# rueberger/MJHMC

Hardware: AMD Instinct MI355X
Metric: particle-steps/sec (ndims x nparticles x L) (higher is better)
Workload: dtype f64 state (ProductOfT: around the f32 matrix-core force)

## Files before the change

### mjhmc_amd/csrc/api.hip

```cpp
#include <hip/hip_runtime.h>

#include <cmath>
#include <cstdio>
#include <functional>
#include <vector>

#include "autocor.hpp"
#include "lagcov.hpp"
#include "sampler_internal.hpp"

static thread_local std::string g_err;

int mjhmc_fail(int code, const std::string& msg) {
  g_err = msg;
  return code;
}
const std::string& last_error_text() { return g_err; }


int pick_shape(int D, int dtype, Shape* out) {
  const int esize = dtype == MJHMC_F64 ? 8 : 4;
  const int VEC = 16 / esize;
  Shape s;
  s.esize = esize;
// ... 467 lines not shown
    if (q) (void)hipFree(q);
  for (void* q : e->sic)
    if (q) (void)hipFree(q);
  delete e;
  return 0;
}

int mjhmc_sampler_destroy(mjhmc_sampler* s) {
  if (!s) return 0;
  (void)hipSetDevice(s->ctx->device);
  if (s->stream) (void)hipStreamSynchronize(s->stream);
  functionals_free_all(s);
  accumulators_free_all(s);
  timegrid_free_all(s);
  stein_free_all(s);
  void* ptrs[] = {s->flf_list, s->call_block, s->Hpre, s->Hwork, s->cold_list, s->pot64_scratch, s->Hspec[0], s->Hspec[1], s->Hspec_dump, s->Gbuf[0], s->Gbuf[1], s->Xbuf[0], s->Xbuf[1], s->Vbuf[0],  s->Vbuf[1], s->EX[0],     s->EX[1],  s->EV[0],
                  s->EV[1],   s->Hflf[0], s->Hflf[1],  s->dwell,  s->dwell_scratch,  s->trans,
                  s->ring,     s->dwell_ring, s->stage,  s->noise,  s->rexp,
                  s->runif,   s->scratch,  s->ck[0],    s->ck[1],    s->ck[2],   s->ck[3],  s->ck[4],
                  s->ck[5],   s->ck[6]};
  for (void* p : ptrs)
    if (p) (void)hipFree(p);
  for (auto& e : s->ev_total)
    if (e) (void)hipEventDestroy(e);
  for (auto& e : s->ev_k) (void)hipEventDestroy(e);
  for (auto& e : s->part_events) (void)hipEventDestroy(e);
  for (auto& q : s->part_streams) (void)hipStreamDestroy(q);
  if (s->ev_join) (void)hipEventDestroy(s->ev_join);
  if (s->ev_fork) (void)hipEventDestroy(s->ev_fork);
  for (void* q : s->ick)
    if (q) (void)hipFree(q);
// ... 44 lines not shown
    const size_t mb = mat_bytes(s);
    for (int i = 0; i < 2; ++i) {
      HIPCHK(hipMalloc(&s->Xbuf[i], mb));
      HIPCHK(hipMalloc(&s->Vbuf[i], mb));
      HIPCHK(hipMemsetAsync(s->Xbuf[i], 0, mb, s->stream));
      HIPCHK(hipMemsetAsync(s->Vbuf[i], 0, mb, s->stream));
      if (e->is_pot() || ((e->is_host() || s->sh.wide) && i == 0)) {
        HIPCHK(hipMalloc(&s->Gbuf[i], mb));
        HIPCHK(hipMemsetAsync(s->Gbuf[i], 0, mb, s->stream));
      }
      if (e->is_dense()) {
        if (!s->Hwork) {
          HIPCHK(hipMalloc((void**)&s->Hwork, s->Npad * ssize(s)));
          HIPCHK(hipMemsetAsync(s->Hwork, 0, s->Npad * ssize(s), s->stream));
          HIPCHK(hipMalloc((void**)&s->cold_list, (2 * s->Npad + 3 * kMaxDenseParts) * sizeof(int)));
          if (e->is_pot() && dtype == MJHMC_F64 && !e->pot_big() && !e->lin_tall())
            HIPCHK(hipMalloc((void**)&s->pot64_scratch, (size_t)kMaxDenseParts * pot64_scratch_workgroups() * 2 * 32 * row_bytes(s)));
        }
        HIPCHK(hipMalloc(&s->Hspec[i], s->Npad * ssize(s)));
        HIPCHK(hipMemsetAsync(s->Hspec[i], 0xFF, s->Npad * ssize(s), s->stream));
      }
      HIPCHK(hipMalloc(&s->EX[i], s->Npad * ssize(s)));
      HIPCHK(hipMalloc(&s->EV[i], s->Npad * ssize(s)));
      HIPCHK(hipMalloc(&s->Hflf[i], s->Npad * ssize(s)));
      HIPCHK(hipMemsetAsync(s->EX[i], 0, s->Npad * ssize(s), s->stream));
      HIPCHK(hipMemsetAsync(s->EV[i], 0, s->Npad * ssize(s), s->stream));
      HIPCHK(hipMemsetAsync(s->Hflf[i], 0xFF, s->Npad * ssize(s), s->stream));
    }
    HIPCHK(hipMalloc((void**)&s->dwell, s->Npad * sizeof(double)));
    HIPCHK(hipMemsetAsync(s->dwell, 0, s->Npad * sizeof(double), s->stream));
    HIPCHK(hipMalloc((void**)&s->dwell_scratch, s->Npad * sizeof(double)));
    HIPCHK(hipMalloc((void**)&s->trans, s->Npad));
// ... 232 lines not shown
```

### mjhmc_amd/csrc/dense_pot.hpp

```cpp
#pragma once
#ifndef __HIPCC_RTC__
#include <hip/hip_runtime.h>
#endif
#include <stdint.h>

#include "jump_math.hpp"
#include "jump_process.hpp"
#include "lane_group.hpp"
#include "philox.hpp"
#include "sampler_args.hpp"

namespace mjhmc {

constexpr int kPotDim = 512;

struct PotModel {
  const float* W1;
  const float* W2T;
  const float* cb;
  const float* alpha;
  int dim;
  int ndims;
};

// ... 142 lines not shown
  hipFunction_t jump32[3][2] = {};
  hipFunction_t jump64[3][2] = {};
  hipFunction_t eval = nullptr, leap = nullptr;
  PotLinear lin{};
};

void pot_launch_jump(const PotJumpArgs& a, const PotModel& mdl, hipStream_t st, const PotGenerated* gen = nullptr);
void pot_launch_eval(const PotEvalArgs& a, const PotModel& mdl, hipStream_t st, const PotGenerated* gen = nullptr);
void pot_launch_leap(const PotLeapArgs& a, const PotModel& mdl, hipStream_t st, const PotGenerated* gen = nullptr);
void pot64_launch_jump(const Pot64JumpArgs& a, const PotModel& mdl, hipStream_t st, const PotGenerated* gen = nullptr);
template <class A>
inline void pot_launch_generated(hipFunction_t f, unsigned grid, hipStream_t st, const A& a, const PotModel& mdl, const PotLinear& lin) {
  void* params[] = {(void*)&a, (void*)&mdl, (void*)&lin};
  (void)hipModuleLaunchKernel(f, grid, 1, 1, 256, 1, 1, 0, st, params, nullptr);
}
int pot64_scratch_workgroups();
#endif

}
```

### mjhmc_amd/csrc/dense_pot64.hip

```cpp
#include <hip/hip_runtime.h>
#include <stdint.h>

#include <algorithm>

#include "dense_pot.hpp"
#include "dense_pot64_kernels.hpp"
#include "dense_pot_tile.hpp"

namespace mjhmc {

__global__ void pot64_cold_list_kernel(const double* __restrict__ Hflf_in, const double* __restrict__ Hspec_in, int64_t N,
                                       int* __restrict__ list, int* __restrict__ count, const Control* ctl) {
  if (ctl->failed) return;
  const int64_t p = (int64_t)blockIdx.x * blockDim.x + threadIdx.x;
  const double hc = p < N ? Hflf_in[p] : 0.0, hs = p < N ? Hspec_in[p] : 0.0;
  append_cold(list, count, (p < N) && !(hc == hc) && !(hs == hs), p);
}

template <int NB, bool REPLAY, int MODE>
__global__ __launch_bounds__(256, 1) void pot64_jump_kernel(const Pot64JumpArgs a, const PotModel mdl) {
  const PotExperts xp;
#include "dense_pot64_jump.inc"
}

// ... 60 lines not shown
  if (n0) atomicAdd(&tally[0], n0);
  if (n1) atomicAdd(&tally[1], n1);
  if (n2) atomicAdd(&tally[2], n2);
  if (n3) atomicAdd(&tally[3], n3);
  __syncthreads();
  if (threadIdx.x < 4 && tally[threadIdx.x]) atomicAdd(&a.stats[threadIdx.x], (unsigned long long)tally[threadIdx.x]);
}

static int resident_cus64() {
  int dev = 0, cus = 0;
  (void)hipGetDevice(&dev);
  (void)hipDeviceGetAttribute(&cus, hipDeviceAttributeMultiprocessorCount, dev);
  return std::max(1, cus);
}

int pot64_scratch_workgroups() { return resident_cus64(); }

template <int NB, int MODE>
static void launch64_mode(const Pot64JumpArgs& a, const PotModel& mdl, unsigned grid, hipStream_t st, const PotGenerated* gen) {
  const bool replay = MODE == kModeControl ? (a.runif && a.noise) : (a.rexp && a.noise);
  if (gen) pot_launch_generated(gen->jump64[MODE][replay ? 1 : 0], grid, st, a, mdl, gen->lin);
  else if (replay) hipLaunchKernelGGL((pot64_jump_kernel<NB, true, MODE>), dim3(grid), dim3(256), 0, st, a, mdl);
  else hipLaunchKernelGGL((pot64_jump_kernel<NB, false, MODE>), dim3(grid), dim3(256), 0, st, a, mdl);
}

template <int NB>
static void launch64_nb(const Pot64JumpArgs& a, const PotModel& mdl, hipStream_t st, const PotGenerated* gen) {
  const int cus = resident_cus64();
  if (a.mode == kModeMJHMC) {
    if (a.iter == 0 || a.rescan) {
      (void)hipMemsetAsync(std::min(a.cold_count, std::min(a.next_count, a.zero_count)), 0, 3 * sizeof(int), st);
      hipLaunchKernelGGL(pot64_cold_list_kernel, dim3((unsigned)((a.N + 255) / 256)), dim3(256), 0, st, a.Hflf_in, a.Hspec_in,
// ... 33 lines not shown
```

### mjhmc_amd/csrc/dense_pot64_jump.inc

```
  __shared__ Shared64<NB> sh;
  if (a.ctl->failed) return;
  const int lane = threadIdx.x & 63, w = threadIdx.x >> 6, c = lane & 31, h = lane >> 5;
  const int ncold = MODE == kModeMJHMC ? *a.cold_count : 0;
  const int64_t nft = (ncold + kP - 1) / kP;
  if ((int64_t)blockIdx.x >= nft + a.ntiles) return;
  if (MODE == kModeMJHMC && blockIdx.x == 0 && threadIdx.x == 0) {
    *a.zero_count = 0;
    if (ncold) atomicAdd(&a.stats[3], (unsigned long long)ncold << 32);
  }
  __shared__ unsigned tally[5];
  if (threadIdx.x < 5) tally[threadIdx.x] = 0;
  AReg<NB> ar;
  areg_load<NB>(mdl, w, c, h, ar);
  stage_bias<NB>(mdl, sh.s);
  const Work<NB> wk = work_of<NB>(a.scratch, blockIdx.x, w, lane);
  for (int64_t item = blockIdx.x; item < nft + a.ntiles; item += gridDim.x) {
    const bool inverse = item < nft;
    [[maybe_unused]] const int istamp_item = (int)(item / gridDim.x) & 15;
    auto column_of = [&](int64_t it) -> int64_t {
      if (it < nft) {
        const int64_t slot = it * kP + c;
        return a.cold_list[slot < ncold ? slot : ncold - 1];
      }
      return (it - nft) * kP + c;
    };
    Tile<NB> g;
    VTile<NB> v;
    float exl = 0.f;
    double EVL;
    {
      const int64_t p = column_of(item);
      POT_ISTAMP(0);
      staged_start<NB>(sh.s, wk, a.X_in, a.V_in, a.G_in, p, w, c, h, g, v, inverse);
      POT_ISTAMP(1);
      EVL = pot64_trajectory<NB>(mdl, xp, ar, sh, w, c, h, lane, wk, g, v, a.L, a.eps, a.chalf, &exl);
      POT_ISTAMP(2);
    }
    int64_t item_again = item;
    asm volatile("" : "+s"(item_again));
    const int64_t p = column_of(item_again);
    const bool alive = p < a.N;
    const size_t roff = (size_t)p * (128 * NB) + 32 * NB * w + 4 * NB * h;
    if (!inverse) staged_end_x<NB>(sh.s, wk, a.X_out, p, w, c, h);
    POT_ISTAMP(3);
    const double EXL = (double)exl;
    const double HL = EXL + EVL;
    if (inverse) {
      if (w == 0 && h == 0) a.Hwork[p] = HL;
      __syncthreads();
      POT_ISTAMP(4);
      continue;
    }

    if constexpr (MODE == kModeMJHMC) {
      if (w == 0 && h == 0) {
        a.EX_out[p] = EXL;
        a.EV_out[p] = EVL;
      }
// ... 54 lines not shown
```

### mjhmc_amd/csrc/dense_pot64_kernels.hpp

```cpp
#pragma once
#ifndef __HIPCC_RTC__
#include <hip/hip_runtime.h>
#endif
#include <stdint.h>

#include "dense_pot.hpp"
#include "dense_pot_tile.hpp"
#include "group_form.hpp"

namespace mjhmc {

template <int NB>
struct DVecN;
template <>
struct DVecN<1> {
  using type = double;
};
template <>
struct DVecN<2> {
  using type = __attribute__((ext_vector_type(2))) double;
};
template <>
struct DVecN<4> {
  using type = __attribute__((ext_vector_type(4))) double;
// ... 16 lines not shown
  return base + (size_t)p * (128 * NB) + 32 * NB * w + 4 * NB * h;
}
template <int NB>
__device__ __forceinline__ double* lane_row(double* base, int64_t p, int w, int h) {
  return base + (size_t)p * (128 * NB) + 32 * NB * w + 4 * NB * h;
}
template <int NB>
__device__ __forceinline__ typename DVecN<NB>::type dv_load(const double* lrow, int q) {
  return *reinterpret_cast<const typename DVecN<NB>::type*>(lrow + q_off<NB>(q));
}
template <int NB>
__device__ __forceinline__ void dv_store(double* lrow, int q, const typename DVecN<NB>::type& v) {
  *reinterpret_cast<typename DVecN<NB>::type*>(lrow + q_off<NB>(q)) = v;
}

constexpr int kPark = 8;
template <int NB>
struct Shared64 {
  Shared<NB> s;
  double red64[4][kP];
  double zn[128 * NB];
  f32x4 park[kPark / 2][256];
};

template <int NB>
struct Work {
  static constexpr int PB = NB == 1 ? 8 : 16;
  static constexpr int PQ = NB * 8 / PB;
  static constexpr unsigned kArea = 16u * PQ * 64u * PB;
  __amdgpu_buffer_rsrc_t rs;
  unsigned voff;
  static constexpr unsigned xb = 0;
  static constexpr unsigned vb = 4 * kArea;
};
template <int NB>
__device__ __forceinline__ Work<NB> work_of(double* scratch, unsigned wg, int w, int lane) {
  Work<NB> k;
  char* base = (char*)scratch + (size_t)wg * (8 * Work<NB>::kArea);
  k.rs = __builtin_amdgcn_make_buffer_rsrc((void*)base, 0, 8 * Work<NB>::kArea, 0x00020000);
  k.voff = (unsigned)w * Work<NB>::kArea + (unsigned)lane * Work<NB>::PB;
  return k;
}
using uvec4 = __attribute__((ext_vector_type(4))) unsigned;
using uvec2 = __attribute__((ext_vector_type(2))) unsigned;
using f64x2 = __attribute__((ext_vector_type(2))) double;
template <int NB>
__device__ __forceinline__ typename DVecN<NB>::type wk_load(const Work<NB>& k, unsigned area, int q) {
  if constexpr (NB == 1) {
    return __builtin_bit_cast(double, __builtin_amdgcn_raw_buffer_load_b64(k.rs, k.voff, area + (unsigned)q * 512u, 0));
  } else if constexpr (NB == 2) {
    return __builtin_bit_cast(f64x2, __builtin_amdgcn_raw_buffer_load_b128(k.rs, k.voff, area + (unsigned)q * 1024u, 0));
  } else {
    const f64x2 lo = __builtin_bit_cast(f64x2, __builtin_amdgcn_raw_buffer_load_b128(k.rs, k.voff, area + (unsigned)q * 2048u, 0));
    const f64x2 hi = __builtin_bit_cast(f64x2, __builtin_amdgcn_raw_buffer_load_b128(k.rs, k.voff, area + (unsigned)q * 2048u + 1024u, 0));
    typename DVecN<4>::type v;
    v[0] = lo[0];
    v[1] = lo[1];
    v[2] = hi[0];
    v[3] = hi[1];
    return v;
  }
}
template <int NB>
__device__ __forceinline__ void wk_store(const Work<NB>& k, unsigned area, int q, const typename DVecN<NB>::type& v) {
  if constexpr (NB == 1) {
    __builtin_amdgcn_raw_buffer_store_b64(__builtin_bit_cast(uvec2, v), k.rs, k.voff, area + (unsigned)q * 512u, 0);
  } else if constexpr (NB == 2) {
    __builtin_amdgcn_raw_buffer_store_b128(__builtin_bit_cast(uvec4, v), k.rs, k.voff, area + (unsigned)q * 1024u, 0);
  } else {
    f64x2 lo, hi;
    lo[0] = v[0];
    lo[1] = v[1];
    hi[0] = v[2];
    hi[1] = v[3];
    __builtin_amdgcn_raw_buffer_store_b128(__builtin_bit_cast(uvec4, lo), k.rs, k.voff, area + (unsigned)q * 2048u, 0);
    __builtin_amdgcn_raw_buffer_store_b128(__builtin_bit_cast(uvec4, hi), k.rs, k.voff, area + (unsigned)q * 2048u + 1024u, 0);
  }
}

template <int NB>
struct PieceOf {
  using type = uvec4;
};
template <>
struct PieceOf<1> {
  using type = unsigned long long;
};
template <int NB>
struct Stage {
  using P = typename PieceOf<NB>::type;
  static constexpr int PB = sizeof(P);
  static constexpr int RB = 1024 * NB;
  static constexpr int RP = RB / PB;
  static constexpr int K = 32 * RP / 256;
  static constexpr int KB = K < 16 ? K : 16;
};
__device__ __forceinline__ unsigned stage_addr(int row, int piece, int pb, int rb) {
  return (unsigned)(row * rb + ((piece ^ (row & 15)) * pb));
}
template <int NB>
__device__ __forceinline__ void stage_rows_in(const double* rows, int64_t p, char* img) {
  using S = Stage<NB>;
  using P = typename S::P;
  const int t = threadIdx.x;
#pragma unroll 1
  for (int i0 = 0; i0 < S::K; i0 += S::KB) {
    P buf[S::KB];
#pragma unroll
    for (int i = 0; i < S::KB; ++i) {
      const int k = (i0 + i) * 256 + t, row = k / S::RP, piece = k % S::RP;
      const int64_t pr = __shfl((long long)p, row);
      buf[i] = *reinterpret_cast<const P*>(reinterpret_cast<const char*>(rows) + (size_t)pr * S::RB + (size_t)piece * S::PB);
    }
#pragma unroll
    for (int i = 0; i < S::KB; ++i) {
      const int k = (i0 + i) * 256 + t, row = k / S::RP, piece = k % S::RP;
      *reinterpret_cast<P*>(img + stage_addr(row, piece, S::PB, S::RB)) = buf[i];
    }
  }
}
template <int NB>
__device__ __forceinline__ void stage_rows_out(double* rows, int64_t p, const char* img) {
  using S = Stage<NB>;
  using P = typename S::P;
  const int t = threadIdx.x;
#pragma unroll 1
  for (int i0 = 0; i0 < S::K; i0 += S::KB) {
#pragma unroll
    for (int i = 0; i < S::KB; ++i) {
      const int k = (i0 + i) * 256 + t, row = k / S::RP, piece = k % S::RP;
      const int64_t pr = __shfl((long long)p, row);
      *reinterpret_cast<P*>(reinterpret_cast<char*>(rows) + (size_t)pr * S::RB + (size_t)piece * S::PB) =
          *reinterpret_cast<const P*>(img + stage_addr(row, piece, S::PB, S::RB));
    }
  }
}
template <int NB>
__device__ __forceinline__ typename DVecN<NB>::type stage_get(const char* img, int w, int c, int h, int q) {
  using S = Stage<NB>;
  const int first = (8 * NB * (32 * w + acc_row(q, h))) / S::PB;
// ... 26 lines not shown
    *reinterpret_cast<typename DVecN<NB>::type*>(img + stage_addr(c, first, S::PB, S::RB)) = v;
  }
}
template <int NB>
__device__ __forceinline__ char* stage_image(Shared<NB>& s) {
  static_assert(sizeof(s.pub) == 32 * Stage<NB>::RB, "the staging image is the two B-operand images");
  return reinterpret_cast<char*>(&s.pub[0][0]);
}

template <int NB>
struct VTile {
  double b[NB][16];
};

template <int NB, int NKICK>
__device__ __forceinline__ void kick_drift_pass(const Work<NB>& wk, const Tile<NB>& g, VTile<NB>& v, double c, double eps,
                                                PubWave<NB>* pub0, int w, int lane) {
  using DV = typename DVecN<NB>::type;
  DV xa[4], xb[4];
  auto load4 = [&](int q4, DV(&x)[4]) {
#pragma unroll
    for (int qq = 0; qq < 4; ++qq) x[qq] = wk_load<NB>(wk, wk.xb, 4 * q4 + qq);
  };
  auto kick4 = [&](int q4) {
#pragma unroll
    for (int qq = 0; qq < 4; ++qq) {
      const int q = 4 * q4 + qq;
#pragma unroll
      for (int r = 0; r < NB; ++r) {
        const double t = c * (double)g.b[r][q];
        double vv = v.b[r][q];
        vv = vv + t;
        if constexpr (NKICK == 2) vv = vv + t;
        v.b[r][q] = vv;
      }
    }
  };
  auto drift4 = [&](int q4, DV(&x)[4]) {
    f32x4 px[NB];
#pragma unroll
    for (int qq = 0; qq < 4; ++qq) {
      const int q = 4 * q4 + qq;
#pragma unroll
      for (int r = 0; r < NB; ++r) {
        const double xx = dget<NB>(x[qq], r) + eps * v.b[r][q];
        dset<NB>(x[qq], r, xx);
        px[r][qq] = (float)xx;
      }
      wk_store<NB>(wk, wk.xb, q, x[qq]);
    }
    if constexpr (NB == 4) {
      unsigned off = ((wk.voff >> 1) & 0xFFFFC000u) | (wk.voff & 0x3FFu);
      asm volatile("" : "+v"(off));
      char* img = reinterpret_cast<char*>(pub0) + off;
#pragma unroll
      for (int r = 0; r < NB; ++r) *reinterpret_cast<f32x4*>(img + (size_t)(r * 4 + q4) * 1024) = px[r];
    } else {
#pragma unroll
      for (int r = 0; r < NB; ++r) pub0[w].v[r][q4][lane] = px[r];
    }
  };
  load4(0, xa);
  load4(1, xb);
  __builtin_amdgcn_sched_barrier(0);
  kick4(0);
  drift4(0, xa);
  __builtin_amdgcn_sched_barrier(0);
  load4(2, xa);
  __builtin_amdgcn_sched_barrier(0);
  kick4(1);
  drift4(1, xb);
  __builtin_amdgcn_sched_barrier(0);
  load4(3, xb);
  __builtin_amdgcn_sched_barrier(0);
  kick4(2);
  drift4(2, xa);
  __builtin_amdgcn_sched_barrier(0);
  kick4(3);
  drift4(3, xb);
}

template <int NB>
__device__ __forceinline__ double closing_kick(const Tile<NB>& g, VTile<NB>& v, double c) {
  double s = 0.0;
#pragma unroll
  for (int q = 0; q < 16; ++q)
#pragma unroll
    for (int r = 0; r < NB; ++r) {
      const double vv = v.b[r][q] + c * (double)g.b[r][q];
      v.b[r][q] = vv;
      s = s + vv * vv;
    }
  return s;
}

template <int NB, class SH>
__device__ __forceinline__ double column_sum(SH& sh, int w, int c, int h, double part) {
  const double both = swap32_sum(part);
  if (h == 0) sh.red64[w][c] = both;
  __syncthreads();
  const double tot = sh.red64[0][c] + sh.red64[1][c] + sh.red64[2][c] + sh.red64[3][c];
  __syncthreads();
  return tot;
}

template <int NB>
__device__ __forceinline__ void staged_start(Shared<NB>& s, const Work<NB>& wk, const double* xin, const double* vin,
                                             const double* gin, int64_t p, int w, int c, int h, Tile<NB>& g, VTile<NB>& v,
                                             bool neg) {
  char* img = stage_image<NB>(s);
  stage_rows_in<NB>(xin, p, img);
  __syncthreads();
#pragma unroll
  for (int q = 0; q < 16; ++q) wk_store<NB>(wk, wk.xb, q, stage_get<NB>(img, w, c, h, q));
  __syncthreads();
  stage_rows_in<NB>(gin, p, img);
  __syncthreads();
#pragma unroll
  for (int q = 0; q < 16; ++q) {
    const typename DVecN<NB>::type gg = stage_get<NB>(img, w, c, h, q);
#pragma unroll
    for (int r = 0; r < NB; ++r) g.b[r][q] = (float)dget<NB>(gg, r);
  }
  __syncthreads();
  stage_rows_in<NB>(vin, p, img);
  __syncthreads();
#pragma unroll
  for (int q = 0; q < 16; ++q) {
    const typename DVecN<NB>::type vv = stage_get<NB>(img, w, c, h, q);
#pragma unroll
    for (int r = 0; r < NB; ++r) v.b[r][q] = neg ? -dget<NB>(vv, r) : dget<NB>(vv, r);
  }
  __syncthreads();
}

template <int NB>
__device__ __forceinline__ void staged_end_x(Shared<NB>& s, const Work<NB>& wk, double* xout, int64_t p, int w, int c, int h) {
  char* img = stage_image<NB>(s);
#pragma unroll
  for (int q = 0; q < 16; ++q) stage_put<NB>(img, w, c, h, q, wk_load<NB>(wk, wk.xb, q));
  __syncthreads();
  stage_rows_out<NB>(xout, p, img);
  __syncthreads();
}
template <int NB>
__device__ __forceinline__ void staged_end_vg(Shared<NB>& s, double* vout, double* gout, int64_t p, int w, int c, int h,
                                              const VTile<NB>& v, const Tile<NB>& g) {
  using DV = typename DVecN<NB>::type;
  char* img = stage_image<NB>(s);
#pragma unroll
  for (int q = 0; q < 16; ++q) {
    DV vv;
#pragma unroll
    for (int r = 0; r < NB; ++r) dset<NB>(vv, r, v.b[r][q]);
    stage_put<NB>(img, w, c, h, q, vv);
  }
  __syncthreads();
  stage_rows_out<NB>(vout, p, img);
  __syncthreads();
#pragma unroll
  for (int q = 0; q < 16; ++q) {
    DV gg;
#pragma unroll
    for (int r = 0; r < NB; ++r) dset<NB>(gg, r, (double)g.b[r][q]);
    stage_put<NB>(img, w, c, h, q, gg);
  }
  __syncthreads();
  stage_rows_out<NB>(gout, p, img);
  __syncthreads();
}

template <int NB, class XP>
__device__ __forceinline__ double pot64_trajectory(const PotModel& mdl, const XP& xp, AReg<NB>& ar, Shared64<NB>& sh, int w, int c, int h,
                                                   int lane, const Work<NB>& wk, Tile<NB>& g, VTile<NB>& v, int L, double eps,
                                                   double chalf, float* ex) {
  PubWave<NB>* pub0 = sh.s.pub[0];
  kick_drift_pass<NB, 1>(wk, g, v, chalf, eps, pub0, w, lane);
  for (int s = 0; s < L; ++s) {
    [[maybe_unused]] const int stamp_slot = s;
    POT_STAMP(0);
    if constexpr (NB == 4) {
#pragma unroll
      for (int k = 0; k < kPark / 2; ++k) {
        f64x2 two;
        two[0] = v.b[NB - 1][15 - 2 * k];
        two[1] = v.b[NB - 1][14 - 2 * k];
        sh.park[k][threadIdx.x] = __builtin_bit_cast(f32x4, two);
      }
    }
    pot_gradient_published<NB>(mdl, xp, ar, sh.s, w, c, h, lane, g, s == L - 1, ex, s);
    if constexpr (NB == 4) {
#pragma unroll
      for (int k = 0; k < kPark / 2; ++k) {
        const f64x2 two = __builtin_bit_cast(f64x2, sh.park[k][threadIdx.x]);
        v.b[NB - 1][15 - 2 * k] = two[0];
        v.b[NB - 1][14 - 2 * k] = two[1];
      }
#pragma unroll
      for (int r = 0; r < NB; ++r)
#pragma unroll
        for (int q = 0; q < 16; ++q) use_here(v.b[r][q]);
    }
    POT_STAMP(6);
    if (s < L - 1) kick_drift_pass<NB, 2>(wk, g, v, chalf, eps, pub0, w, lane);
    POT_STAMP(7);
  }
  const double part = closing_kick<NB>(g, v, chalf);
  return column_sum<NB>(sh, w, c, h, part) / 2.0;
}


template <int NB>
struct Finish64Shared {
  struct {
    int move[kP];
  } s;
  double red64[4][kP];
  double zn[128 * NB];
};
// ... 142 lines not shown
```

### mjhmc_amd/csrc/dense_pot_tile.hpp

```cpp
#pragma once
#ifndef __HIPCC_RTC__
#include <hip/hip_runtime.h>
#endif
#include <stdint.h>

#include "dense_pot.hpp"
#include "timing_variants.hpp"

namespace mjhmc {

using f32x16 = __attribute__((ext_vector_type(16))) float;
using f32x4 = __attribute__((ext_vector_type(4))) float;

constexpr int kP = 32;

__device__ __forceinline__ int acc_row(int q, int h) { return (q & 3) + 8 * (q >> 2) + 4 * h; }

template <int NB>
struct Tile {
  f32x16 b[NB];
};

template <int NB>
struct VecN;
// ... 54 lines not shown
template <int NB>
__device__ __forceinline__ void publish(PubWave<NB>& dst, int lane, const Tile<NB>& t) {
#pragma unroll
  for (int r = 0; r < NB; ++r)
#pragma unroll
    for (int q4 = 0; q4 < 4; ++q4) {
      f32x4 v;
      v[0] = t.b[r][4 * q4 + 0];
      v[1] = t.b[r][4 * q4 + 1];
      v[2] = t.b[r][4 * q4 + 2];
      v[3] = t.b[r][4 * q4 + 3];
      dst.v[r][q4][lane] = v;
    }
}

template <int NB>
__device__ __forceinline__ void a_chunk_load(const float* mlane, int chunk, typename VecN<NB>::type (&dst)[16]) {
  using V = typename VecN<NB>::type;
  constexpr int DIM = 128 * NB;
  const float* base = mlane + (size_t)(32 * NB * (chunk / NB) + (chunk % NB)) * DIM;
#pragma unroll
  for (int q = 0; q < 16; ++q) dst[q] = *reinterpret_cast<const V*>(base + (size_t)(NB * ((q & 3) + 8 * (q >> 2))) * DIM);
}

template <int NB>
__device__ __forceinline__ typename VecN<NB>::type buf_load(__amdgpu_buffer_rsrc_t r, unsigned voff, unsigned soff) {
  using V = typename VecN<NB>::type;
  if constexpr (NB == 4) return __builtin_bit_cast(V, __builtin_amdgcn_raw_buffer_load_b128(r, voff, soff, 0));
  else if constexpr (NB == 2) return __builtin_bit_cast(V, __builtin_amdgcn_raw_buffer_load_b64(r, voff, soff, 0));
  else return __builtin_bit_cast(V, __builtin_amdgcn_raw_buffer_load_b32(r, voff, soff, 0));
}
template <int NB>
__device__ __forceinline__ __amdgpu_buffer_rsrc_t a_rsrc(const float* M) {
  constexpr int DIM = 128 * NB;
  return __builtin_amdgcn_make_buffer_rsrc((void*)M, 0, DIM * DIM * 4, 0x00020000);
}
template <int NB>
// ... 58 lines not shown
  const __amdgpu_buffer_rsrc_t rM = a_rsrc<NB>(M), rN = a_rsrc<NB>(Mnext);
  const f32x4* bbase = &pub[0].v[0][0][0];
  typename VecN<NB>::type a1[16];
  f32x4 bnext = bbase[lane];
#pragma unroll 1
  for (int chunk = 0; chunk < NCH; chunk += 2) {
    const bool more = chunk + 2 < NCH;
    const int c1 = chunk + 1, c2 = more ? chunk + 2 : 0;
    chunk_mfma_ld<NB>(bbase, chunk, lane, a0, bnext, acc, rM, lane_bytes,
                      (unsigned)(32 * NB * (c1 / NB) + (c1 % NB)) * (unsigned)(DIM * 4), a1);
    chunk_mfma_ld<NB>(bbase, chunk + 1, lane, a1, bnext, acc, more ? rM : rN, lane_bytes,
                      (unsigned)(32 * NB * (c2 / NB) + (c2 % NB)) * (unsigned)(DIM * 4), a0);
  }
}

template <int NB>
struct AReg {
  typename VecN<NB>::type a0[16];
};
template <>
struct AReg<1> {
  float w1[4][16];
  float w2[4][16];
};

template <int NB>
__device__ __forceinline__ void areg_load(const PotModel& mdl, int w, int c, int h, AReg<NB>& ar) {
  if constexpr (NB == 1) {
    const float* m1 = mdl.W1 + (size_t)(4 * h) * 128 + 32 * w + c;
    const float* m2 = mdl.W2T + (size_t)(4 * h) * 128 + 32 * w + c;
#pragma unroll
    for (int chunk = 0; chunk < 4; ++chunk) {
      a_chunk_load<1>(m1, chunk, ar.w1[chunk]);
      a_chunk_load<1>(m2, chunk, ar.w2[chunk]);
    }
  } else {
    a_chunk_load<NB>(mdl.W1 + (size_t)(4 * NB * h) * (128 * NB) + 32 * NB * w + NB * c, 0, ar.a0);
  }
}

template <int NB, bool SECOND>
__device__ __forceinline__ void gemm_any(const PotModel& mdl, AReg<NB>& ar, const PubWave<NB>* pub, int w, int c,
                                         int h, int lane, Tile<NB>& acc) {
  if constexpr (NB == 1) {
    const int kdim = mdl.ndims;
#pragma unroll
    for (int chunk = 0; chunk < 4; ++chunk) {
      const float(&a)[16] = SECOND ? ar.w2[chunk] : ar.w1[chunk];
      const f32x4(*blk)[64] = pub[chunk].v[0];
#pragma unroll
      for (int q4 = 0; q4 < 4; ++q4) {
        if (32 * chunk + 8 * q4 < kdim) {
          const f32x4 b4 = blk[q4][lane];
#pragma unroll
          for (int qq = 0; qq < 4; ++qq)
            acc.b[0] = __builtin_amdgcn_mfma_f32_32x32x2f32(a[4 * q4 + qq], b4[qq], acc.b[0], 0, 0, 0);
        }
      }
    }
  } else {
    gemm_dim<NB>(SECOND ? mdl.W2T : mdl.W1, SECOND ? mdl.W1 : mdl.W2T, pub, w, c, h, lane, ar.a0, acc);
  }
}

template <int NB>
__device__ __forceinline__ void rowvec_load(const float* vec, int w, int h, Tile<NB>& t) {
  using V = typename VecN<NB>::type;
  const float* base = vec + 32 * NB * w;
#pragma unroll
  for (int q = 0; q < 16; ++q) {
    const V v = *reinterpret_cast<const V*>(base + NB * acc_row(q, h));
#pragma unroll
    for (int r = 0; r < NB; ++r) t.b[r][q] = vget<NB>(v, r);
  }
// ... 29 lines not shown
    zn[2 * pair] = 2 * pair < D ? (F)z0 : (F)0;
    zn[2 * pair + 1] = 2 * pair + 1 < D ? (F)z1 : (F)0;
  }
}

template <int NB>
__device__ __forceinline__ void stage_bias(const PotModel& mdl, Shared<NB>& sh) {
  for (int i = threadIdx.x; i < 128 * NB; i += 256) sh.cb[i] = mdl.cb[i];
}


struct PotExperts {
  static constexpr bool kProductOfT = true;
};

template <int NB, class XP>
__device__ __forceinline__ void pot_gradient_published(const PotModel& mdl, const XP& xp, AReg<NB>& ar, Shared<NB>& sh, int w, int c, int h,
                                                       int lane, Tile<NB>& g, bool want_energy, float* energy_out,
                                                       int stamp_slot = 0) {
  __syncthreads();
  POT_STAMP(1);
  Tile<NB> u;
  rowvec_load<NB>(sh.cb, w, h, u);
  gemm_any<NB, false>(mdl, ar, sh.pub[0], w, c, h, lane, u);
  POT_STAMP(2);
  if constexpr (XP::kProductOfT) {
    if (want_energy) {
      using V = typename VecN<NB>::type;
      const float* al = mdl.alpha + 32 * NB * w;
      float s = 0.f;
#pragma unroll
      for (int q = 0; q < 16; ++q) {
// ... 104 lines not shown
```

### mjhmc_amd/csrc/handles.hpp

```cpp
#pragma once
#include <hip/hip_runtime.h>

#include <string>
#include <vector>

#include "../../include/mjhmc_hip.h"
#include "dense_pot.hpp"
#include "dense_sic.hpp"
#include "launcher_decls.hpp"
#include "linear_energy.hpp"
#include "sampler_args.hpp"
#include "user_expr.hpp"

using namespace mjhmc;

int mjhmc_fail(int code, const std::string& msg);

#define HIPCHK(expr)                                                                                         \
  do {                                                                                                       \
    hipError_t e_ = (expr);                                                                                  \
    if (e_ != hipSuccess)                                                                                    \
      return mjhmc_fail(MJHMC_ERR_HIP, std::string(#expr) + ": " + hipGetErrorString(e_) + " (" + __FILE__ + \
                                           ":" + std::to_string(__LINE__) + ")");                            \
  } while (0)
// ... 72 lines not shown
  Shape sh;
  hipStream_t stream = nullptr;
  char* h_pin = nullptr;
  size_t h_pin_cap = 0;
  std::vector<hipStream_t> part_streams;
  std::vector<hipEvent_t> part_events;
  hipEvent_t ev_join = nullptr;
  void* ick[7] = {nullptr, nullptr, nullptr, nullptr, nullptr, nullptr, nullptr};
  hipEvent_t ev_fork = nullptr;
  void* Xbuf[2] = {nullptr, nullptr};
  void* Vbuf[2] = {nullptr, nullptr};
  void* Xcur = nullptr;
  void* Gbuf[2] = {nullptr, nullptr};
  float* Hwork = nullptr;
  int* cold_list = nullptr;
  double* pot64_scratch = nullptr;
  void* Hspec[2] = {nullptr, nullptr};
  void* Hspec_dump = nullptr;
  int* flf_list = nullptr;
  bool list_valid = false;
  int list_par = 0;
  int list_count = 0;
  int* flf_counts = nullptr;
  void* Hpre = nullptr;
  int vcur = 0, scur = 0;
  void* EX[2] = {nullptr, nullptr};
  void* EV[2] = {nullptr, nullptr};
  void* Hflf[2] = {nullptr, nullptr};
  double* dwell = nullptr;
  double* dwell_scratch = nullptr;
  void* ck[7] = {nullptr, nullptr, nullptr, nullptr, nullptr, nullptr, nullptr};
// ... 75 lines not shown
```

### mjhmc_amd/csrc/iterate.hip

```cpp
#include <hip/hip_runtime.h>

#include <atomic>
#include <chrono>
#include <cmath>
#include <cstdio>
#include <type_traits>
#include <vector>

#include "energies.hpp"
#include "sampler_internal.hpp"
#include "schedule.hpp"

constexpr size_t kCtlBytes = 64;
static_assert(sizeof(Control) <= kCtlBytes, "the failure flag's slot of the call block");
static size_t counts_bytes(int cap) { return (((size_t)cap + 1) * sizeof(int) + 63) / 64 * 64; }
int ensure_call_block(mjhmc_sampler* s, int rows) {
  if (s->call_block && s->stats_cap >= rows) return 0;
  const int cap = std::max(rows, 1024);
  if (s->call_block) {
    HIPCHK(hipStreamSynchronize(s->stream));
    HIPCHK(hipFree(s->call_block));
    s->call_block = nullptr;
    s->ctl = nullptr;
    s->flf_counts = nullptr;
// ... 300 lines not shown
  h.dwell_ring = a.dwell_ring + start;
  h.trans = a.trans + start;
  if constexpr (IsDenseJump<A>::value) {
    h.Hspec_in = a.Hspec_in + start;
    h.Hwork = a.Hwork + start;
    h.Hspec_out = a.Hspec_out + start;
    h.cold_list = a.cold_list + start;
    h.next_list = a.next_list + start;
    h.cold_count = counters + 3 * which + a.iter % 3;
    h.next_count = counters + 3 * which + (a.iter + 1) % 3;
    h.zero_count = counters + 3 * which + (a.iter + 2) % 3;
    if constexpr (A::kPot) {
      h.G_in = a.G_in + (size_t)start * pitch;
      h.G_out = a.G_out + (size_t)start * pitch;
    }
    if constexpr (A::kScratch)
      h.scratch = a.scratch + (size_t)which * pot64_scratch_workgroups() * 2 * 32 * (size_t)pitch;
  }
  h.N = n;
  h.Npad = npad;
  h.first_pid = a.first_pid + start;
  return h;
}

static int ensure_part_streams(mjhmc_sampler* s, int n_parts) {
  if (!s->ev_fork) {
    HIPCHK(hipEventCreateWithFlags(&s->ev_fork, hipEventDisableTiming));
    HIPCHK(hipEventCreateWithFlags(&s->ev_join, hipEventDisableTiming));
  }
  while ((int)s->part_streams.size() < n_parts - 1) {
    hipStream_t q;
    hipEvent_t e;
// ... 257 lines not shown
  const int vi = (s->vcur + i) & 1, si = (s->scur + i) & 1;
  A d = jump_args<A>(s, i, vi, si, xin, xout, ring_slot0, s->stats + 4 * i);
  d.noise = rp.normal ? (const S*)s->noise : nullptr;
  d.rexp = rp.exp ? s->rexp : nullptr;
  d.runif = rp.unif ? s->runif : nullptr;
  if constexpr (A::kPot) {
    d.G_in = (const S*)s->Gbuf[vi];
    d.G_out = (S*)s->Gbuf[vi ^ 1];
  }
  d.Hwork = (H*)s->Hwork;
  d.cold_list = s->cold_list + (size_t)(i & 1) * s->Npad;
  d.next_list = s->cold_list + (size_t)((i + 1) & 1) * s->Npad;
  d.Hspec_in = (const H*)s->Hspec[si];
  d.Hspec_out = (H*)(spec_out ? spec_out : s->Hspec[si ^ 1]);
  d.rescan = spec_out ? 1 : 0;
  if constexpr (A::kScratch) d.scratch = s->pot64_scratch;
  for (int k = 0; k < parts.n; ++k) {
    A h = part_args(d, parts.start(k), parts.count(s, k), parts.npad(s, k), (size_t)s->sh.pitch, k, s->cold_list + 2 * s->Npad);
    h.ntiles = dense_ntiles(s, h.N, h.Npad);
    if constexpr (!POT) sic_launch_jump(h, s->en->sic_model(), parts.stream(s, k));
    else if constexpr (sizeof(S) == 8) pot64_launch_jump(h, s->en->pot_model(), parts.stream(s, k), s->en->pot_gen());
    else pot_launch_jump(h, s->en->pot_model(), parts.stream(s, k), s->en->pot_gen());
  }
}

template <typename T>
static int iterate_dense_parts(mjhmc_sampler* s, int n_iter, const Replay& rp, int ring_slot0, mjhmc_iter_stats* per_iter,
                               int* n_done, bool allow_split, bool* run_again) {
  *run_again = false;
  TRY(replay_alloc(s, rp));
  const Parts parts = dense_split(s, allow_split && !rp.any());
// ... 265 lines not shown
```

### mjhmc_amd/csrc/sampler_args.hpp

```cpp
#pragma once
#include <stdint.h>

#include "philox.hpp"

namespace mjhmc {

constexpr int kModeMJHMC = 0;
constexpr int kModeControl = 1;
constexpr int kModeCT = 2;

struct Control {
  int failed;
  int failed_iter;
  int inv_iter;
};

constexpr int kMaxFuse = 64;

constexpr int kAbNoBlockDecide = 1, kAbNoWpp = 2, kAbNoQuad = 4, kAbNoRows = 8, kAbNoRelay = 16, kAbForceRelay = 32;

inline bool fused_rows_shape(int mode, int logG, int ab) {
  return mode == kModeMJHMC && (logG == 1 || logG == 2) && !(ab & kAbNoRows);
}

// ... 116 lines not shown

struct NoField {};
template <bool HAS, typename F>
struct FieldIfT {
  using type = F;
};
template <typename F>
struct FieldIfT<false, F> {
  using type = NoField;
};
template <bool HAS, typename F>
using FieldIf = typename FieldIfT<HAS, F>::type;

template <typename S, typename H, bool POT>
struct DenseJumpArgs {
  static constexpr bool kPot = POT, kScratch = POT && sizeof(S) == 8;
  const S* X_in;
  const S* V_in;
  [[no_unique_address]] FieldIf<POT, const S*> G_in;
  S* X_out;
  S* V_out;
  [[no_unique_address]] FieldIf<POT, S*> G_out;
  const H* EX_in;
  const H* EV_in;
  const H* Hflf_in;
  H* Hwork;
  int* cold_list;
  int* cold_count;
  int* next_list;
  int* next_count;
  int* zero_count;
  int rescan;
  const H* Hspec_in;
  H* Hspec_out;
  H* EX_out;
  H* EV_out;
  H* Hflf_out;
  double* dwell;
  double* dwell_ring;
  uint8_t* trans;
  const S* noise;
  const double* rexp;
  const double* runif;
  [[no_unique_address]] FieldIf<kScratch, double*> scratch;
  Control* ctl;
  unsigned long long* stats;
  int64_t N, Npad, ntiles, first_pid;
  [[no_unique_address]] FieldIf<POT, int> D;
  int L, iter;
  int mode;
  H eps, chalf, r_keep, r_mix;
  double p_r, p_flip;
  RngKey key;
};

template <typename S, bool POT>
struct DenseLeapArgs {
  const S* X;
  const S* V;
// ... 43 lines not shown
```

Baseline: 62.02 billion.

## Keep f64 positions in registers and halve resident A-weight registers in pot64 kernel

```diff
diff --git a/mjhmc_amd/csrc/api.hip b/mjhmc_amd/csrc/api.hip
--- a/mjhmc_amd/csrc/api.hip
+++ b/mjhmc_amd/csrc/api.hip
@@ -505,7 +505,7 @@
   accumulators_free_all(s);
   timegrid_free_all(s);
   stein_free_all(s);
-  void* ptrs[] = {s->flf_list, s->call_block, s->Hpre, s->Hwork, s->cold_list, s->pot64_scratch, s->Hspec[0], s->Hspec[1], s->Hspec_dump, s->Gbuf[0], s->Gbuf[1], s->Xbuf[0], s->Xbuf[1], s->Vbuf[0],  s->Vbuf[1], s->EX[0],     s->EX[1],  s->EV[0],
+  void* ptrs[] = {s->flf_list, s->call_block, s->Hpre, s->Hwork, s->cold_list, s->Hspec[0], s->Hspec[1], s->Hspec_dump, s->Gbuf[0], s->Gbuf[1], s->Xbuf[0], s->Xbuf[1], s->Vbuf[0],  s->Vbuf[1], s->EX[0],     s->EX[1],  s->EV[0],
                   s->EV[1],   s->Hflf[0], s->Hflf[1],  s->dwell,  s->dwell_scratch,  s->trans,
                   s->ring,     s->dwell_ring, s->stage,  s->noise,  s->rexp,
                   s->runif,   s->scratch,  s->ck[0],    s->ck[1],    s->ck[2],   s->ck[3],  s->ck[4],
@@ -580,8 +580,6 @@
           HIPCHK(hipMalloc((void**)&s->Hwork, s->Npad * ssize(s)));
           HIPCHK(hipMemsetAsync(s->Hwork, 0, s->Npad * ssize(s), s->stream));
           HIPCHK(hipMalloc((void**)&s->cold_list, (2 * s->Npad + 3 * kMaxDenseParts) * sizeof(int)));
-          if (e->is_pot() && dtype == MJHMC_F64 && !e->pot_big() && !e->lin_tall())
-            HIPCHK(hipMalloc((void**)&s->pot64_scratch, (size_t)kMaxDenseParts * pot64_scratch_workgroups() * 2 * 32 * row_bytes(s)));
         }
         HIPCHK(hipMalloc(&s->Hspec[i], s->Npad * ssize(s)));
         HIPCHK(hipMemsetAsync(s->Hspec[i], 0xFF, s->Npad * ssize(s), s->stream));
diff --git a/mjhmc_amd/csrc/dense_pot.hpp b/mjhmc_amd/csrc/dense_pot.hpp
--- a/mjhmc_amd/csrc/dense_pot.hpp
+++ b/mjhmc_amd/csrc/dense_pot.hpp
@@ -180,7 +180,6 @@
   void* params[] = {(void*)&a, (void*)&mdl, (void*)&lin};
   (void)hipModuleLaunchKernel(f, grid, 1, 1, 256, 1, 1, 0, st, params, nullptr);
 }
-int pot64_scratch_workgroups();
 #endif
 
 }
diff --git a/mjhmc_amd/csrc/dense_pot64.hip b/mjhmc_amd/csrc/dense_pot64.hip
--- a/mjhmc_amd/csrc/dense_pot64.hip
+++ b/mjhmc_amd/csrc/dense_pot64.hip
@@ -98,8 +98,6 @@
   return std::max(1, cus);
 }
 
-int pot64_scratch_workgroups() { return resident_cus64(); }
-
 template <int NB, int MODE>
 static void launch64_mode(const Pot64JumpArgs& a, const PotModel& mdl, unsigned grid, hipStream_t st, const PotGenerated* gen) {
   const bool replay = MODE == kModeControl ? (a.runif && a.noise) : (a.rexp && a.noise);
diff --git a/mjhmc_amd/csrc/dense_pot64_jump.inc b/mjhmc_amd/csrc/dense_pot64_jump.inc
--- a/mjhmc_amd/csrc/dense_pot64_jump.inc
+++ b/mjhmc_amd/csrc/dense_pot64_jump.inc
@@ -10,10 +10,9 @@
   }
   __shared__ unsigned tally[5];
   if (threadIdx.x < 5) tally[threadIdx.x] = 0;
-  AReg<NB> ar;
+  AReg64<NB> ar;
   areg_load<NB>(mdl, w, c, h, ar);
   stage_bias<NB>(mdl, sh.s);
-  const Work<NB> wk = work_of<NB>(a.scratch, blockIdx.x, w, lane);
   for (int64_t item = blockIdx.x; item < nft + a.ntiles; item += gridDim.x) {
     const bool inverse = item < nft;
     [[maybe_unused]] const int istamp_item = (int)(item / gridDim.x) & 15;
@@ -25,15 +24,15 @@
       return (it - nft) * kP + c;
     };
     Tile<NB> g;
-    VTile<NB> v;
+    VTile<NB> v, x;
     float exl = 0.f;
     double EVL;
     {
       const int64_t p = column_of(item);
       POT_ISTAMP(0);
-      staged_start<NB>(sh.s, wk, a.X_in, a.V_in, a.G_in, p, w, c, h, g, v, inverse);
+      staged_start<NB>(sh.s, a.X_in, a.V_in, a.G_in, p, w, c, h, g, v, x, inverse);
       POT_ISTAMP(1);
-      EVL = pot64_trajectory<NB>(mdl, xp, ar, sh, w, c, h, lane, wk, g, v, a.L, a.eps, a.chalf, &exl);
+      EVL = pot64_trajectory<NB>(mdl, xp, ar, sh, w, c, h, lane, g, v, x, a.L, a.eps, a.chalf, &exl);
       POT_ISTAMP(2);
     }
     int64_t item_again = item;
@@ -41,7 +40,7 @@
     const int64_t p = column_of(item_again);
     const bool alive = p < a.N;
     const size_t roff = (size_t)p * (128 * NB) + 32 * NB * w + 4 * NB * h;
-    if (!inverse) staged_end_x<NB>(sh.s, wk, a.X_out, p, w, c, h);
+    if (!inverse) staged_end_x<NB>(sh.s, a.X_out, p, w, c, h, x);
     POT_ISTAMP(3);
     const double EXL = (double)exl;
     const double HL = EXL + EVL;
diff --git a/mjhmc_amd/csrc/dense_pot64_kernels.hpp b/mjhmc_amd/csrc/dense_pot64_kernels.hpp
--- a/mjhmc_amd/csrc/dense_pot64_kernels.hpp
+++ b/mjhmc_amd/csrc/dense_pot64_kernels.hpp
@@ -54,6 +54,11 @@
   *reinterpret_cast<typename DVecN<NB>::type*>(lrow + q_off<NB>(q)) = v;
 }
 
+template <int NB>
+constexpr int kA64 = NB == 4 ? 8 : 16;
+template <int NB>
+using AReg64 = AReg<NB, kA64<NB>>;
+
 constexpr int kPark = 8;
 template <int NB>
 struct Shared64 {
@@ -63,60 +68,8 @@
   f32x4 park[kPark / 2][256];
 };
 
-template <int NB>
-struct Work {
-  static constexpr int PB = NB == 1 ? 8 : 16;
-  static constexpr int PQ = NB * 8 / PB;
-  static constexpr unsigned kArea = 16u * PQ * 64u * PB;
-  __amdgpu_buffer_rsrc_t rs;
-  unsigned voff;
-  static constexpr unsigned xb = 0;
-  static constexpr unsigned vb = 4 * kArea;
-};
-template <int NB>
-__device__ __forceinline__ Work<NB> work_of(double* scratch, unsigned wg, int w, int lane) {
-  Work<NB> k;
-  char* base = (char*)scratch + (size_t)wg * (8 * Work<NB>::kArea);
-  k.rs = __builtin_amdgcn_make_buffer_rsrc((void*)base, 0, 8 * Work<NB>::kArea, 0x00020000);
-  k.voff = (unsigned)w * Work<NB>::kArea + (unsigned)lane * Work<NB>::PB;
-  return k;
-}
 using uvec4 = __attribute__((ext_vector_type(4))) unsigned;
-using uvec2 = __attribute__((ext_vector_type(2))) unsigned;
 using f64x2 = __attribute__((ext_vector_type(2))) double;
-template <int NB>
-__device__ __forceinline__ typename DVecN<NB>::type wk_load(const Work<NB>& k, unsigned area, int q) {
-  if constexpr (NB == 1) {
-    return __builtin_bit_cast(double, __builtin_amdgcn_raw_buffer_load_b64(k.rs, k.voff, area + (unsigned)q * 512u, 0));
-  } else if constexpr (NB == 2) {
-    return __builtin_bit_cast(f64x2, __builtin_amdgcn_raw_buffer_load_b128(k.rs, k.voff, area + (unsigned)q * 1024u, 0));
-  } else {
-    const f64x2 lo = __builtin_bit_cast(f64x2, __builtin_amdgcn_raw_buffer_load_b128(k.rs, k.voff, area + (unsigned)q * 2048u, 0));
-    const f64x2 hi = __builtin_bit_cast(f64x2, __builtin_amdgcn_raw_buffer_load_b128(k.rs, k.voff, area + (unsigned)q * 2048u + 1024u, 0));
-    typename DVecN<4>::type v;
-    v[0] = lo[0];
-    v[1] = lo[1];
-    v[2] = hi[0];
-    v[3] = hi[1];
-    return v;
-  }
-}
-template <int NB>
-__device__ __forceinline__ void wk_store(const Work<NB>& k, unsigned area, int q, const typename DVecN<NB>::type& v) {
-  if constexpr (NB == 1) {
-    __builtin_amdgcn_raw_buffer_store_b64(__builtin_bit_cast(uvec2, v), k.rs, k.voff, area + (unsigned)q * 512u, 0);
-  } else if constexpr (NB == 2) {
-    __builtin_amdgcn_raw_buffer_store_b128(__builtin_bit_cast(uvec4, v), k.rs, k.voff, area + (unsigned)q * 1024u, 0);
-  } else {
-    f64x2 lo, hi;
-    lo[0] = v[0];
-    lo[1] = v[1];
-    hi[0] = v[2];
-    hi[1] = v[3];
-    __builtin_amdgcn_raw_buffer_store_b128(__builtin_bit_cast(uvec4, lo), k.rs, k.voff, area + (unsigned)q * 2048u, 0);
-    __builtin_amdgcn_raw_buffer_store_b128(__builtin_bit_cast(uvec4, hi), k.rs, k.voff, area + (unsigned)q * 2048u + 1024u, 0);
-  }
-}
 
 template <int NB>
 struct PieceOf {
@@ -126,6 +79,10 @@
 struct PieceOf<1> {
   using type = unsigned long long;
 };
+__device__ __forceinline__ int here(int lane_const) {
+  asm volatile("" : "+v"(lane_const));
+  return lane_const;
+}
 template <int NB>
 struct Stage {
   using P = typename PieceOf<NB>::type;
@@ -142,7 +99,7 @@
 __device__ __forceinline__ void stage_rows_in(const double* rows, int64_t p, char* img) {
   using S = Stage<NB>;
   using P = typename S::P;
-  const int t = threadIdx.x;
+  const int t = here(threadIdx.x);
 #pragma unroll 1
   for (int i0 = 0; i0 < S::K; i0 += S::KB) {
     P buf[S::KB];
@@ -163,7 +120,7 @@
 __device__ __forceinline__ void stage_rows_out(double* rows, int64_t p, const char* img) {
   using S = Stage<NB>;
   using P = typename S::P;
-  const int t = threadIdx.x;
+  const int t = here(threadIdx.x);
 #pragma unroll 1
   for (int i0 = 0; i0 < S::K; i0 += S::KB) {
 #pragma unroll
@@ -220,15 +177,11 @@
 };
 
 template <int NB, int NKICK>
-__device__ __forceinline__ void kick_drift_pass(const Work<NB>& wk, const Tile<NB>& g, VTile<NB>& v, double c, double eps,
+__device__ __forceinline__ void kick_drift_pass(const Tile<NB>& g, VTile<NB>& v, VTile<NB>& x, double c, double eps,
                                                 PubWave<NB>* pub0, int w, int lane) {
-  using DV = typename DVecN<NB>::type;
-  DV xa[4], xb[4];
-  auto load4 = [&](int q4, DV(&x)[4]) {
-#pragma unroll
-    for (int qq = 0; qq < 4; ++qq) x[qq] = wk_load<NB>(wk, wk.xb, 4 * q4 + qq);
-  };
-  auto kick4 = [&](int q4) {
+#pragma unroll
+  for (int q4 = 0; q4 < 4; ++q4) {
+    f32x4 px[NB];
 #pragma unroll
     for (int qq = 0; qq < 4; ++qq) {
       const int q = 4 * q4 + qq;
@@ -239,51 +192,15 @@
         vv = vv + t;
         if constexpr (NKICK == 2) vv = vv + t;
         v.b[r][q] = vv;
-      }
-    }
-  };
-  auto drift4 = [&](int q4, DV(&x)[4]) {
-    f32x4 px[NB];
-#pragma unroll
-    for (int qq = 0; qq < 4; ++qq) {
-      const int q = 4 * q4 + qq;
-#pragma unroll
-      for (int r = 0; r < NB; ++r) {
-        const double xx = dget<NB>(x[qq], r) + eps * v.b[r][q];
-        dset<NB>(x[qq], r, xx);
+        const double xx = x.b[r][q] + eps * vv;
+        x.b[r][q] = xx;
         px[r][qq] = (float)xx;
       }
-      wk_store<NB>(wk, wk.xb, q, x[qq]);
-    }
-    if constexpr (NB == 4) {
-      unsigned off = ((wk.voff >> 1) & 0xFFFFC000u) | (wk.voff & 0x3FFu);
-      asm volatile("" : "+v"(off));
-      char* img = reinterpret_cast<char*>(pub0) + off;
-#pragma unroll
-      for (int r = 0; r < NB; ++r) *reinterpret_cast<f32x4*>(img + (size_t)(r * 4 + q4) * 1024) = px[r];
-    } else {
-#pragma unroll
-      for (int r = 0; r < NB; ++r) pub0[w].v[r][q4][lane] = px[r];
-    }
-  };
-  load4(0, xa);
-  load4(1, xb);
-  __builtin_amdgcn_sched_barrier(0);
-  kick4(0);
-  drift4(0, xa);
-  __builtin_amdgcn_sched_barrier(0);
-  load4(2, xa);
-  __builtin_amdgcn_sched_barrier(0);
-  kick4(1);
-  drift4(1, xb);
-  __builtin_amdgcn_sched_barrier(0);
-  load4(3, xb);
-  __builtin_amdgcn_sched_barrier(0);
-  kick4(2);
-  drift4(2, xa);
-  __builtin_amdgcn_sched_barrier(0);
-  kick4(3);
-  drift4(3, xb);
+    }
+#pragma unroll
+    for (int r = 0; r < NB; ++r) pub0[w].v[r][q4][lane] = px[r];
+    __builtin_amdgcn_sched_barrier(0);
+  }
 }
 
 template <int NB>
@@ -311,14 +228,18 @@
 }
 
 template <int NB>
-__device__ __forceinline__ void staged_start(Shared<NB>& s, const Work<NB>& wk, const double* xin, const double* vin,
-                                             const double* gin, int64_t p, int w, int c, int h, Tile<NB>& g, VTile<NB>& v,
-                                             bool neg) {
+__device__ __forceinline__ void staged_start(Shared<NB>& s, const double* xin, const double* vin, const double* gin, int64_t p,
+                                             int w, int c, int h, Tile<NB>& g, VTile<NB>& v, VTile<NB>& x, bool neg) {
   char* img = stage_image<NB>(s);
+  c = here(c), w = here(w), h = here(h);
   stage_rows_in<NB>(xin, p, img);
   __syncthreads();
 #pragma unroll
-  for (int q = 0; q < 16; ++q) wk_store<NB>(wk, wk.xb, q, stage_get<NB>(img, w, c, h, q));
+  for (int q = 0; q < 16; ++q) {
+    const typename DVecN<NB>::type xx = stage_get<NB>(img, w, c, h, q);
+#pragma unroll
+    for (int r = 0; r < NB; ++r) x.b[r][q] = dget<NB>(xx, r);
+  }
   __syncthreads();
   stage_rows_in<NB>(gin, p, img);
   __syncthreads();
@@ -341,10 +262,16 @@
 }
 
 template <int NB>
-__device__ __forceinline__ void staged_end_x(Shared<NB>& s, const Work<NB>& wk, double* xout, int64_t p, int w, int c, int h) {
+__device__ __forceinline__ void staged_end_x(Shared<NB>& s, double* xout, int64_t p, int w, int c, int h, const VTile<NB>& x) {
   char* img = stage_image<NB>(s);
-#pragma unroll
-  for (int q = 0; q < 16; ++q) stage_put<NB>(img, w, c, h, q, wk_load<NB>(wk, wk.xb, q));
+  c = here(c), w = here(w), h = here(h);
+#pragma unroll
+  for (int q = 0; q < 16; ++q) {
+    typename DVecN<NB>::type xx;
+#pragma unroll
+    for (int r = 0; r < NB; ++r) dset<NB>(xx, r, x.b[r][q]);
+    stage_put<NB>(img, w, c, h, q, xx);
+  }
   __syncthreads();
   stage_rows_out<NB>(xout, p, img);
   __syncthreads();
@@ -354,6 +281,7 @@
                                               const VTile<NB>& v, const Tile<NB>& g) {
   using DV = typename DVecN<NB>::type;
   char* img = stage_image<NB>(s);
+  c = here(c), w = here(w), h = here(h);
 #pragma unroll
   for (int q = 0; q < 16; ++q) {
     DV vv;
@@ -377,11 +305,11 @@
 }
 
 template <int NB, class XP>
-__device__ __forceinline__ double pot64_trajectory(const PotModel& mdl, const XP& xp, AReg<NB>& ar, Shared64<NB>& sh, int w, int c, int h,
-                                                   int lane, const Work<NB>& wk, Tile<NB>& g, VTile<NB>& v, int L, double eps,
+__device__ __forceinline__ double pot64_trajectory(const PotModel& mdl, const XP& xp, AReg64<NB>& ar, Shared64<NB>& sh, int w, int c, int h,
+                                                   int lane, Tile<NB>& g, VTile<NB>& v, VTile<NB>& x, int L, double eps,
                                                    double chalf, float* ex) {
   PubWave<NB>* pub0 = sh.s.pub[0];
-  kick_drift_pass<NB, 1>(wk, g, v, chalf, eps, pub0, w, lane);
+  kick_drift_pass<NB, 1>(g, v, x, chalf, eps, pub0, w, lane);
   for (int s = 0; s < L; ++s) {
     [[maybe_unused]] const int stamp_slot = s;
     POT_STAMP(0);
@@ -408,7 +336,7 @@
         for (int q = 0; q < 16; ++q) use_here(v.b[r][q]);
     }
     POT_STAMP(6);
-    if (s < L - 1) kick_drift_pass<NB, 2>(wk, g, v, chalf, eps, pub0, w, lane);
+    if (s < L - 1) kick_drift_pass<NB, 2>(g, v, x, chalf, eps, pub0, w, lane);
     POT_STAMP(7);
   }
   const double part = closing_kick<NB>(g, v, chalf);
diff --git a/mjhmc_amd/csrc/dense_pot_tile.hpp b/mjhmc_amd/csrc/dense_pot_tile.hpp
--- a/mjhmc_amd/csrc/dense_pot_tile.hpp
+++ b/mjhmc_amd/csrc/dense_pot_tile.hpp
@@ -92,13 +92,13 @@
     }
 }
 
-template <int NB>
-__device__ __forceinline__ void a_chunk_load(const float* mlane, int chunk, typename VecN<NB>::type (&dst)[16]) {
+template <int NB, int AQ = 16>
+__device__ __forceinline__ void a_chunk_load(const float* mlane, int chunk, typename VecN<NB>::type (&dst)[AQ]) {
   using V = typename VecN<NB>::type;
   constexpr int DIM = 128 * NB;
   const float* base = mlane + (size_t)(32 * NB * (chunk / NB) + (chunk % NB)) * DIM;
 #pragma unroll
-  for (int q = 0; q < 16; ++q) dst[q] = *reinterpret_cast<const V*>(base + (size_t)(NB * ((q & 3) + 8 * (q >> 2))) * DIM);
+  for (int q = 0; q < AQ; ++q) dst[q] = *reinterpret_cast<const V*>(base + (size_t)(NB * ((q & 3) + 8 * (q >> 2))) * DIM);
 }
 
 template <int NB>
@@ -187,18 +187,64 @@
   }
 }
 
-template <int NB>
+template <int NB, int HALF, int NHALF>
+__device__ __forceinline__ void half_mfma_ld(const f32x4* bbase, int chunk, int lane, const typename VecN<NB>::type (&a)[8],
+                                             f32x4& bnext, Tile<NB>& acc, __amdgpu_buffer_rsrc_t rs, unsigned lane_bytes,
+                                             unsigned cbase, typename VecN<NB>::type (&aload)[8]) {
+  constexpr int NG = 16 * NB, DIM = 128 * NB;
+#pragma unroll
+  for (int q4 = 2 * HALF; q4 < 2 * HALF + 2; ++q4) {
+    const f32x4 b4 = bnext;
+    const int t = 4 * chunk + q4 + 1;
+    bnext = bbase[(size_t)(t < NG ? t : NG - 1) * 64 + lane];
+    __builtin_amdgcn_sched_barrier(0);
+#pragma unroll
+    for (int qq = 0; qq < 4; ++qq) {
+      const int j = 4 * (q4 - 2 * HALF) + qq, qn = 8 * NHALF + j;
+#pragma unroll
+      for (int r = 0; r < NB; ++r)
+        acc.b[r] = __builtin_amdgcn_mfma_f32_32x32x2f32(vget<NB>(a[j], r), b4[qq], acc.b[r], 0, 0, 0);
+      aload[j] = buf_load<NB>(rs, lane_bytes, cbase + (unsigned)(NB * ((qn & 3) + 8 * (qn >> 2)) * DIM * 4));
+      __builtin_amdgcn_sched_barrier(0);
+    }
+    __builtin_amdgcn_sched_barrier(0);
+  }
+}
+
+template <int NB>
+__device__ __forceinline__ void gemm_dim_half(const float* __restrict__ M, const float* __restrict__ Mnext, const PubWave<NB>* pub,
+                                              int w, int c, int h, int lane, typename VecN<NB>::type (&a0)[8], Tile<NB>& acc) {
+  constexpr int DIM = 128 * NB, NCH = 4 * NB;
+  const size_t lane_off = (size_t)(4 * NB * h) * DIM + 32 * NB * w + NB * c;
+  const unsigned lane_bytes = (unsigned)(lane_off * sizeof(float));
+  const __amdgpu_buffer_rsrc_t rM = a_rsrc<NB>(M), rN = a_rsrc<NB>(Mnext);
+  const f32x4* bbase = &pub[0].v[0][0][0];
+  typename VecN<NB>::type a1[8];
+  f32x4 bnext = bbase[lane];
+  auto cbase_of = [](int ch) { return (unsigned)(32 * NB * (ch / NB) + (ch % NB)) * (unsigned)(DIM * 4); };
+#pragma unroll 1
+  for (int chunk = 0; chunk < NCH; chunk += 2) {
+    const bool more = chunk + 2 < NCH;
+    const int c1 = chunk + 1, c2 = more ? chunk + 2 : 0;
+    half_mfma_ld<NB, 0, 1>(bbase, chunk, lane, a0, bnext, acc, rM, lane_bytes, cbase_of(chunk), a1);
+    half_mfma_ld<NB, 1, 0>(bbase, chunk, lane, a1, bnext, acc, rM, lane_bytes, cbase_of(c1), a0);
+    half_mfma_ld<NB, 0, 1>(bbase, c1, lane, a0, bnext, acc, rM, lane_bytes, cbase_of(c1), a1);
+    half_mfma_ld<NB, 1, 0>(bbase, c1, lane, a1, bnext, acc, more ? rM : rN, lane_bytes, cbase_of(c2), a0);
+  }
+}
+
+template <int NB, int AQ = 16>
 struct AReg {
-  typename VecN<NB>::type a0[16];
-};
-template <>
-struct AReg<1> {
+  typename VecN<NB>::type a0[AQ];
+};
+template <int AQ>
+struct AReg<1, AQ> {
   float w1[4][16];
   float w2[4][16];
 };
 
-template <int NB>
-__device__ __forceinline__ void areg_load(const PotModel& mdl, int w, int c, int h, AReg<NB>& ar) {
+template <int NB, int AQ>
+__device__ __forceinline__ void areg_load(const PotModel& mdl, int w, int c, int h, AReg<NB, AQ>& ar) {
   if constexpr (NB == 1) {
     const float* m1 = mdl.W1 + (size_t)(4 * h) * 128 + 32 * w + c;
     const float* m2 = mdl.W2T + (size_t)(4 * h) * 128 + 32 * w + c;
@@ -208,12 +254,12 @@
       a_chunk_load<1>(m2, chunk, ar.w2[chunk]);
     }
   } else {
-    a_chunk_load<NB>(mdl.W1 + (size_t)(4 * NB * h) * (128 * NB) + 32 * NB * w + NB * c, 0, ar.a0);
-  }
-}
-
-template <int NB, bool SECOND>
-__device__ __forceinline__ void gemm_any(const PotModel& mdl, AReg<NB>& ar, const PubWave<NB>* pub, int w, int c,
+    a_chunk_load<NB, AQ>(mdl.W1 + (size_t)(4 * NB * h) * (128 * NB) + 32 * NB * w + NB * c, 0, ar.a0);
+  }
+}
+
+template <int NB, bool SECOND, int AQ>
+__device__ __forceinline__ void gemm_any(const PotModel& mdl, AReg<NB, AQ>& ar, const PubWave<NB>* pub, int w, int c,
                                          int h, int lane, Tile<NB>& acc) {
   if constexpr (NB == 1) {
     const int kdim = mdl.ndims;
@@ -231,6 +277,8 @@
         }
       }
     }
+  } else if constexpr (AQ == 8) {
+    gemm_dim_half<NB>(SECOND ? mdl.W2T : mdl.W1, SECOND ? mdl.W1 : mdl.W2T, pub, w, c, h, lane, ar.a0, acc);
   } else {
     gemm_dim<NB>(SECOND ? mdl.W2T : mdl.W1, SECOND ? mdl.W1 : mdl.W2T, pub, w, c, h, lane, ar.a0, acc);
   }
@@ -290,8 +338,8 @@
   static constexpr bool kProductOfT = true;
 };
 
-template <int NB, class XP>
-__device__ __forceinline__ void pot_gradient_published(const PotModel& mdl, const XP& xp, AReg<NB>& ar, Shared<NB>& sh, int w, int c, int h,
+template <int NB, class XP, int AQ>
+__device__ __forceinline__ void pot_gradient_published(const PotModel& mdl, const XP& xp, AReg<NB, AQ>& ar, Shared<NB>& sh, int w, int c, int h,
                                                        int lane, Tile<NB>& g, bool want_energy, float* energy_out,
                                                        int stamp_slot = 0) {
   __syncthreads();
diff --git a/mjhmc_amd/csrc/handles.hpp b/mjhmc_amd/csrc/handles.hpp
--- a/mjhmc_amd/csrc/handles.hpp
+++ b/mjhmc_amd/csrc/handles.hpp
@@ -110,7 +110,6 @@
   void* Gbuf[2] = {nullptr, nullptr};
   float* Hwork = nullptr;
   int* cold_list = nullptr;
-  double* pot64_scratch = nullptr;
   void* Hspec[2] = {nullptr, nullptr};
   void* Hspec_dump = nullptr;
   int* flf_list = nullptr;
diff --git a/mjhmc_amd/csrc/iterate.hip b/mjhmc_amd/csrc/iterate.hip
--- a/mjhmc_amd/csrc/iterate.hip
+++ b/mjhmc_amd/csrc/iterate.hip
@@ -338,8 +338,6 @@
       h.G_in = a.G_in + (size_t)start * pitch;
       h.G_out = a.G_out + (size_t)start * pitch;
     }
-    if constexpr (A::kScratch)
-      h.scratch = a.scratch + (size_t)which * pot64_scratch_workgroups() * 2 * 32 * (size_t)pitch;
   }
   h.N = n;
   h.Npad = npad;
@@ -627,7 +625,6 @@
   d.Hspec_in = (const H*)s->Hspec[si];
   d.Hspec_out = (H*)(spec_out ? spec_out : s->Hspec[si ^ 1]);
   d.rescan = spec_out ? 1 : 0;
-  if constexpr (A::kScratch) d.scratch = s->pot64_scratch;
   for (int k = 0; k < parts.n; ++k) {
     A h = part_args(d, parts.start(k), parts.count(s, k), parts.npad(s, k), (size_t)s->sh.pitch, k, s->cold_list + 2 * s->Npad);
     h.ntiles = dense_ntiles(s, h.N, h.Npad);
diff --git a/mjhmc_amd/csrc/sampler_args.hpp b/mjhmc_amd/csrc/sampler_args.hpp
--- a/mjhmc_amd/csrc/sampler_args.hpp
+++ b/mjhmc_amd/csrc/sampler_args.hpp
@@ -154,7 +154,7 @@
 
 template <typename S, typename H, bool POT>
 struct DenseJumpArgs {
-  static constexpr bool kPot = POT, kScratch = POT && sizeof(S) == 8;
+  static constexpr bool kPot = POT;
   const S* X_in;
   const S* V_in;
   [[no_unique_address]] FieldIf<POT, const S*> G_in;
@@ -182,7 +182,6 @@
   const S* noise;
   const double* rexp;
   const double* runif;
-  [[no_unique_address]] FieldIf<kScratch, double*> scratch;
   Control* ctl;
   unsigned long long* stats;
   int64_t N, Npad, ntiles, first_pid;
```

Measured after the change: 63.14 billion (median of 6 runs). 1.8% higher.
